# dioph/periodicity

Hardware: AMD Instinct MI355X
Metric: Lomb-Scargle Gpair/s (sample x freq), fp64, N=1e5 x 1e6 per GPU (higher is better)
Workload: dtype f64

## Files before the change

periodicity_amd/csrc/gls.hip:

```cpp
#include "pdc_internal.h"
#include "gls_epilogue.h"
#include "gls_sums.h"

#include <cstdlib>

using namespace pdc;

namespace {

constexpr int kBlock = 256;
constexpr int kPrepBlock = 1024;

enum Mode { MODE_FIT_MEAN = 0, MODE_NO_MEAN = 1, MODE_RAW = 2, MODE_TREND = 3 };
constexpr bool mode_fits_mean(int m) { return m == MODE_FIT_MEAN; }
constexpr bool mode_sums_w(int m) { return m == MODE_FIT_MEAN || m == MODE_TREND; }

struct TrendScalars {
    double W;
    double yy, y1, ty, tt, t1;
    double shift;
    double inv_span;
    double prec_a, prec_alpha, prec_beta;
    double log_const;
};
// ... 45 lines not shown
    const int64_t off = a.offsets ? a.offsets[blockIdx.x] : 0;
    const int64_t n = a.offsets ? a.offsets[blockIdx.x + 1] - off : a.n_total;
    const double *t = a.shared_t ? a.t : a.t + off;
    const int32_t *pk = a.picks ? a.picks + off : nullptr;
    const double *y = pk ? a.y : a.y + off;
    const double *dy = a.dy ? (pk ? a.dy : a.dy + off) : nullptr;
    auto at = [pk](int64_t i) -> int64_t { return pk ? (int64_t)pk[i] : i; };
    double *rec = a.rec + off * 6;
    const double t0 = n > 0 ? t[0] : 0.0;

    double W = 1.0, ybar = 0.0;
    if (!a.raw) {
        double acc = 0.0;
        for (int64_t i = tid; i < n; i += kPrepBlock) {
            const double e = dy ? dy[at(i)] : 1.0;
            acc += 1.0 / (e * e);
        }
        W = block_sum<kPrepBlock>(acc, red);
        if (a.fit_mean) {
            acc = 0.0;
            for (int64_t i = tid; i < n; i += kPrepBlock) {
                const double e = dy ? dy[at(i)] : 1.0;
                acc += (1.0 / (e * e)) / W * y[at(i)];
            }
            ybar = block_sum<kPrepBlock>(acc, red);
        }
    }
    double yy = 0.0, wsum = 0.0;
    if (a.rw) {
        for (int64_t i = tid; i < n; i += kPrepBlock) {
            const double e = dy ? dy[at(i)] : 1.0;
            const double w = (1.0 / (e * e)) / W;
            const double yc = y[at(i)] - ybar;
            const double wy = w * yc;
            yy += wy * yc;
            wsum += w;
            if (dy) reinterpret_cast<double2 *>(a.rw)[i * a.bpad + blockIdx.x] = make_double2(wy, w);
            else a.rw[i * a.bpad + blockIdx.x] = wy;
            if (blockIdx.x == 0) a.tp[i] = t[i] - t0;
        }
    } else
    for (int64_t i = tid; i < n; i += kPrepBlock) {
        const double tp = t[i] - t0;
        double w, wy;
        if (a.raw) {
            w = y[at(i)];
            wy = w;
        } else {
            const double e = dy ? dy[at(i)] : 1.0;
            w = (1.0 / (e * e)) / W;
            const double yc = y[at(i)] - ybar;
            wy = w * yc;
            yy += wy * yc;
            wsum += w;
        }
        double sd, cd;
        sincos_cycles(frac_product(a.delta, tp), sd, cd);
        if (!a.raw) {
            w = sqrt(w);
            wy = w * (y[at(i)] - ybar);
        }
        double2 *r = reinterpret_cast<double2 *>(rec + i * 6);
        r[0] = make_double2(wy, w);
        r[1] = make_double2(cd, sd);
        r[2] = make_double2(cd + cd, tp);
    }
    yy = block_sum<kPrepBlock>(yy, red);
    wsum = block_sum<kPrepBlock>(wsum, red);
    if (tid == 0) {
        double *s = a.scal + (int64_t)blockIdx.x * 4;
        s[0] = yy;
        s[1] = wsum;
        s[2] = W;
        s[3] = t0;
    }
}

constexpr int kPrepParts = 512;

struct WidePrepArgs {
    PrepArgs p;
    int nparts;
    double *part;
};

__global__ __launch_bounds__(kBlock) void gls_prep_wide_a(WidePrepArgs a) {
    __shared__ double red[kBlock / 64];
    double sw = 0.0, swy = 0.0;
    for (int64_t i = (int64_t)blockIdx.x * kBlock + threadIdx.x; i < a.p.n_total;
         i += (int64_t)gridDim.x * kBlock) {
        const double wr = inv_var(a.p.dy, i);
        sw += wr;
        swy += wr * a.p.y[i];
    }
    sw = block_sum<kBlock>(sw, red);
    swy = block_sum<kBlock>(swy, red);
    if (threadIdx.x == 0) {
        a.part[blockIdx.x] = sw;
        a.part[kPrepParts + blockIdx.x] = swy;
    }
}

__device__ __forceinline__ double fold_partials(const double *p, int count, double *red) {
    double v = 0.0;
    for (int i = threadIdx.x; i < count; i += kBlock) v += p[i];
    return block_sum<kBlock>(v, red);
}

__global__ __launch_bounds__(kBlock) void gls_prep_wide_b(WidePrepArgs a) {
    __shared__ double red[kBlock / 64];
    const double W = fold_partials(a.part, a.nparts, red);
    const double ybar = a.p.fit_mean ? fold_partials(a.part + kPrepParts, a.nparts, red) / W : 0.0;
    const double t0 = a.p.t[0];
    double yy = 0.0, wsum = 0.0;
    for (int64_t i = (int64_t)blockIdx.x * kBlock + threadIdx.x; i < a.p.n_total;
         i += (int64_t)gridDim.x * kBlock) {
        const double tp = a.p.t[i] - t0;
        const double w = inv_var(a.p.dy, i) / W;
        const double yc = a.p.y[i] - ybar;
        const double wy = w * yc;
        yy += wy * yc;
        wsum += w;
        double sd, cd;
        sincos_cycles(frac_product(a.p.delta, tp), sd, cd);
        const double rw = sqrt(w);
        double2 *r = reinterpret_cast<double2 *>(a.p.rec + i * 6);
        r[0] = make_double2(rw * yc, rw);
        r[1] = make_double2(cd, sd);
        r[2] = make_double2(cd + cd, tp);
    }
    yy = block_sum<kBlock>(yy, red);
    wsum = block_sum<kBlock>(wsum, red);
    if (threadIdx.x == 0) {
        a.part[2 * kPrepParts + blockIdx.x] = yy;
        a.part[3 * kPrepParts + blockIdx.x] = wsum;
    }
}

__global__ __launch_bounds__(kBlock) void gls_prep_wide_c(WidePrepArgs a) {
    __shared__ double red[kBlock / 64];
    const double W = fold_partials(a.part, a.nparts, red);
    const double yy = fold_partials(a.part + 2 * kPrepParts, a.nparts, red);
    const double wsum = fold_partials(a.part + 3 * kPrepParts, a.nparts, red);
    if (threadIdx.x == 0) {
        a.p.scal[0] = yy;
        a.p.scal[1] = wsum;
        a.p.scal[2] = W;
        a.p.scal[3] = a.p.t[0];
    }
}

constexpr int kPairM = 8;
constexpr int kPairRow = kPairM * 4;

__global__ __launch_bounds__(kBlock) void gls_pair_table_kernel(const double *rec, double *tab, int64_t n_total, double delta) {
    const int64_t g = (int64_t)blockIdx.x * kBlock + threadIdx.x;
    const int64_t i = g / kPairM;
    if (i >= n_total + 2) return;
    double c = 0.0, s = 0.0, c2 = 0.0, s2 = 0.0;
    if (i < n_total) {
        const double tp = rec[i * 6 + 5];
        const double k = (double)(2 * (int)(g % kPairM) + 1), h = 0.5 * delta;
        const double hi = h * tp, lo = __builtin_fma(h, tp, -hi);
        const double p = k * hi, pe = __builtin_fma(k, hi, -p);
        const double r = (p - __builtin_rint(p)) + __builtin_fma(k, lo, pe);
        sincos_cycles(r, s, c);
        sincos_cycles(r + r, s2, c2);
    }
    double2 *o = reinterpret_cast<double2 *>(tab + g * 4);
    o[0] = make_double2(c, s);
    o[1] = make_double2(c2, s2);
}

template <int MODE>
__device__ __forceinline__ double gls_power(double Sh, double Ch, double S, double C, double SS,
                                            double SC, double YY, double Wsum, double Werr,
                                            int psd) {
    const double S2 = 2.0 * SC;
    const double C2 = Wsum - 2.0 * SS;
    return gls_power_from_sums<mode_fits_mean(MODE)>(Sh, Ch, S, C, S2, C2, YY, Werr, psd);
}

__device__ __forceinline__ double bglst_loglik(double Sh, double Ch, double S, double C, double SS, double SC,
                                               double TS, double TC, double Wsum, const TrendScalars &q) {
    const double tc = TC * q.inv_span + q.shift * C, ts = TS * q.inv_span + q.shift * S;
    const double W = q.W;
    const double m00 = W * (Wsum - SS) + q.prec_a;
    const double m10 = W * SC, m11 = W * SS + q.prec_a;
    const double m20 = W * tc, m21 = W * ts, m22 = W * q.tt + q.prec_alpha;
    const double m30 = W * C, m31 = W * S, m32 = W * q.t1, m33 = W * Wsum + q.prec_beta;
    const double b0 = W * Ch, b1 = W * Sh, b2 = W * q.ty, b3 = W * q.y1;
    const double l00 = __builtin_sqrt(m00);
    const double l10 = m10 / l00, l20 = m20 / l00, l30 = m30 / l00;
    const double l11 = __builtin_sqrt(m11 - l10 * l10);
    const double l21 = (m21 - l20 * l10) / l11, l31 = (m31 - l30 * l10) / l11;
    const double l22 = __builtin_sqrt(m22 - l20 * l20 - l21 * l21);
    const double l32 = (m32 - l30 * l20 - l31 * l21) / l22;
    const double l33 = __builtin_sqrt(m33 - l30 * l30 - l31 * l31 - l32 * l32);
    const double z0 = b0 / l00;
    const double z1 = (b1 - l10 * z0) / l11;
    const double z2 = (b2 - l20 * z0 - l21 * z1) / l22;
    const double z3 = (b3 - l30 * z0 - l31 * z1 - l32 * z2) / l33;
    const double quad = W * q.yy - (z0 * z0 + z1 * z1 + z2 * z2 + z3 * z3);
    const double logdet = 2.0 * (log(l00) + log(l11) + log(l22) + log(l33));
    return -0.5 * (quad + logdet + q.log_const);
}

template <int K, int MODE, int SPLIT, bool BAL = false, bool PAIR = false>
__global__ __launch_bounds__(kBlock, (K >= 16 ? 2 : 1)) void gls_scan_kernel(GlsArgs a) {
    static_assert(!PAIR || (K == 2 * kPairM && (MODE == MODE_FIT_MEAN || MODE == MODE_NO_MEAN)), "mirrored pairs: K = 16, the two GLS modes");
    constexpr int FT = kBlock / SPLIT;
    constexpr bool TIGHT = BAL || K >= 16;
    constexpr int COLS = FT / 64;
    constexpr int kChunk = SPLIT == 1 ? 64 : 128;
    __shared__ double2 tab[kChunk + 1][COLS * 8 + 8 + 1];
    __shared__ double red_v[4];
    __shared__ long long red_i[4];
    __shared__ double2 sc_k[6];
    __shared__ double gf_red[PAIR ? 16 : 1][16];
    __shared__ double gf_acc[16];
    const int tid_ = threadIdx.x;
    if (TIGHT && tid_ < 6) sc_k[tid_] = sincos_coefficient(tid_);

    const int64_t G = BAL ? a.bal_slots : a.n_curves * a.tiles;
    const int64_t per_xcd = (G + 7) / 8;
    int64_t L = (int64_t)(blockIdx.x % 8) * per_xcd + blockIdx.x / 8;
    int zpart = blockIdx.y;
    if (a.parts_by_xcd) {
        const int64_t q = blockIdx.x / 8, zi = q / G;
        L = q - zi * G;
        zpart = (int)(blockIdx.x % 8) + 8 * (int)zi;
        if (zpart >= a.parts) return;
    }
    if (L >= G) return;
    int64_t bal_u = 0, bal_hi = 0;
    if (BAL) {
        bal_u = L * a.bal_units / a.bal_slots;
        bal_hi = (L + 1) * a.bal_units / a.bal_slots;
        if (bal_u >= bal_hi) return;
    }
    do {
    int64_t curve = L / a.tiles;
    int64_t tile = L - curve * a.tiles;
    int64_t bal_take = 0;
    int bal_piece = 0;
    int64_t bal_c0 = 0;
    if (BAL) {
        curve = 0;
        int64_t b_chunks = a.bal_chunks, b_slots = a.bal_slots, b_units = a.bal_units;
        asm volatile("" : "+s"(b_chunks), "+s"(b_slots), "+s"(b_units));
        tile = (bal_hi - 1) / b_chunks;
        const int64_t t0 = tile * b_chunks;
        bal_c0 = (bal_u > t0 ? bal_u : t0) - t0;
        bal_take = bal_hi - t0 - bal_c0;
        int64_t s_of = t0 * b_slots / b_units;
        while ((s_of + 1) * b_units / b_slots <= t0) ++s_of;
        while (s_of * b_units / b_slots > t0) --s_of;
        bal_piece = (int)(L - s_of);
    }

    const int64_t off = a.offsets ? a.offsets[curve] : 0;
    const int64_t n = a.offsets ? a.offsets[curve + 1] - off : a.n_total;
    const int wave = __builtin_amdgcn_readfirstlane(tid_ >> 6), part = wave % SPLIT;
    const int col = wave / SPLIT;
    const int64_t jt = tile * FT * (int64_t)K;
    const int64_t jl = jt + (col * 64 + (tid_ & 63)) * (int64_t)K;
    const double f_tile = __dadd_rn(a.f0, __dmul_rn((double)(a.j_begin + jt), a.delta));
    const double kdelta = (double)K * a.delta;

    static_assert(MODE != MODE_TREND || (SPLIT == 1 && !BAL && K <= 8), "BGLST: eight sums per frequency, whole curves per tile");
    double Sh[K], Ch[K], S[K], C[K], SS[K], SC[K];
    double TS[K], TC[K];
#pragma unroll
    for (int k = 0; k < K; ++k) Sh[k] = Ch[k] = S[k] = C[k] = SS[k] = SC[k] = TS[k] = TC[k] = 0.0;
    if (PAIR) {
        int t16 = tid_;
        asm volatile("" : "+v"(t16));
        if (t16 < 16) gf_acc[t16] = 0.0;
    }

    const int64_t s_begin = BAL ? bal_c0 * kChunk : (a.partial ? (int64_t)zpart * a.z_len : 0);
    const int64_t s_stop = BAL ? s_begin + bal_take * kChunk : s_begin + a.z_len;
    const int64_t s_end = (BAL || a.partial) ? (s_stop < n ? s_stop : n) : n;
    for (int64_t base = s_begin; base < s_end; base += kChunk) {
        __syncthreads();
        int tid = tid_;
        if (TIGHT) asm volatile("" : "+v"(tid));
        const int lane = tid & 63;
        const int slot_a = col * 8 + (lane >> 3), slot_b = COLS * 8 + (lane & 7);
        if (PAIR) {
            constexpr int SPP = kChunk / 16;
            const int m16 = tid & 15, seg = tid >> 4;
            const int64_t i0 = base + seg * SPP;
            const double *tp_ = a.pair_tab + (off + i0) * kPairRow + (m16 & 7) * 4 + (m16 < 8 ? 1 : 3);
            const double *rp_ = a.rec + (off + i0) * 6 + 1;
            double acc = 0.0;
#pragma unroll
            for (int q = 0; q < SPP; ++q) {
                const bool live = i0 + q < s_end;
                const double sq = live ? rp_[q * 6] : 0.0;
                const double v = live ? tp_[q * kPairRow] : 0.0;
                acc = __builtin_fma(sq * sq, m16 < 8 ? v * v : v, acc);
            }
            gf_red[seg][m16] = acc;
            __builtin_amdgcn_sched_barrier(0);
        }
        if (tid < 2 * kChunk) {
            const int il = tid >> 1;
            const bool live = base + il < s_end;
            const double tp = live ? a.rec[(off + base + il) * 6 + 5] : 0.0;
            const double sqw = live ? a.rec[(off + base + il) * 6 + 1] : 0.0;
            double2 step1, cur;
            double2 kk[6];
            if (TIGHT) {
#pragma unroll
                for (int q = 0; q < 6; ++q) kk[q] = sc_k[q];
            }
            auto sincos_fill = [&](const double r, double &s_, double &c_) {
                if (TIGHT) sincos_cycles_k(r, kk, s_, c_);
                else sincos_cycles(r, s_, c_);
            };
            if ((tid & 1) == 0) {
                sincos_fill(frac_product(kdelta, tp), step1.x, step1.y);
                double one = 1.0, zero = 0.0;
                if (TIGHT) asm volatile("" : "+v"(one), "+v"(zero));
                tab[il][COLS * 8] = make_double2(zero, one);
                tab[il][COLS * 8 + 1] = step1;
                cur = step1;
#pragma unroll
                for (int q = 2; q < 8; ++q) {
                    cur = rot2(cur, step1);
                    tab[il][COLS * 8 + q] = cur;
                }
                double r_base = frac_product(f_tile, tp);
                if (PAIR) {
                    double dl = a.delta;
                    asm volatile("" : "+v"(dl));
                    r_base += frac_product(8.0 * dl, tp) - frac_product(0.5 * dl, tp);
                }
                sincos_fill(r_base, cur.x, cur.y);
                if (MODE == MODE_FIT_MEAN || MODE == MODE_NO_MEAN || MODE == MODE_TREND) {
                    cur.x *= sqw;
                    cur.y *= sqw;
                }
            } else {
                sincos_fill(frac_product(8.0 * kdelta, tp), step1.x, step1.y);
            }
            double2 b0;
            b0.x = __shfl_xor(cur.x, 1, 64);
            b0.y = __shfl_xor(cur.y, 1, 64);
            if (tid & 1) {
                tab[il][0] = b0;
#pragma unroll
                for (int q = 1; q < COLS * 8; ++q) {
                    b0 = rot2(b0, step1);
                    tab[il][q] = b0;
                }
            }
        }
        __syncthreads();
        const int cnt = (int)((s_end - base) < kChunk ? (s_end - base) : kChunk);
        const int i_end = cnt < (part + 1) * (kChunk / SPLIT) ? cnt : (part + 1) * (kChunk / SPLIT);
        const int i_beg = part * (kChunk / SPLIT);
        if constexpr (PAIR) {
            if (tid < 16) {
                double g = gf_red[0][tid];
#pragma unroll
                for (int q = 1; q < 16; ++q) g += gf_red[q][tid];
                gf_acc[tid] += g;
            }
            using d8 = double __attribute__((ext_vector_type(8)));
            using cd8 = __attribute__((address_space(4))) const d8;
            using d2 = double __attribute__((ext_vector_type(2)));
            using cd2 = __attribute__((address_space(4))) const d2;
            auto uniform = [](const double *p) {
                const uintptr_t u = reinterpret_cast<uintptr_t>(p);
                const uint32_t lo_ = __builtin_amdgcn_readfirstlane((uint32_t)u), hi_ = __builtin_amdgcn_readfirstlane((uint32_t)(u >> 32));
                return ((uintptr_t)hi_ << 32) | lo_;
            };
            const cd8 *stab = reinterpret_cast<const cd8 *>(uniform(a.pair_tab + (off + base) * kPairRow));
            const cd2 *srec = reinterpret_cast<const cd2 *>(uniform(a.rec + (off + base) * 6));
            const int i_last = __builtin_amdgcn_readfirstlane(i_end);
            d8 h0a, h0b, h1a, h1b;
            d2 r;
            double2 qa, qt;
            auto request_first = [&](const int i) {
                h0a = stab[i * 4];
                h0b = stab[i * 4 + 1];
                r = srec[i * 3];
                qa = tab[i][slot_a];
                qt = tab[i][slot_b];
            };
            double A1, B1, A2, B2, a2, ab;
            auto pair_fmas = [&](const d8 &h, const int m0) {
#pragma unroll
                for (int q = 0; q < 2; ++q) {
                    const int hi = K / 2 + m0 + q, lo = K / 2 - 1 - m0 - q;
                    const double c = h[4 * q], s = h[4 * q + 1], c2 = h[4 * q + 2], s2 = h[4 * q + 3];
                    Sh[hi] = __builtin_fma(c, A1, Sh[hi]);
                    Sh[lo] = __builtin_fma(s, B1, Sh[lo]);
                    Ch[hi] = __builtin_fma(c, B1, Ch[hi]);
                    Ch[lo] = __builtin_fma(s, A1, Ch[lo]);
                    if (mode_sums_w(MODE)) {
                        S[hi] = __builtin_fma(c, A2, S[hi]);
                        S[lo] = __builtin_fma(s, B2, S[lo]);
                        C[hi] = __builtin_fma(c, B2, C[hi]);
                        C[lo] = __builtin_fma(s, A2, C[lo]);
                    }
                    SS[hi] = __builtin_fma(c2, a2, SS[hi]);
                    SS[lo] = __builtin_fma(s2, ab, SS[lo]);
                    SC[hi] = __builtin_fma(c2, ab, SC[hi]);
                    SC[lo] = __builtin_fma(s2, a2, SC[lo]);
                }
            };
            if (i_beg < i_last) {
                request_first(i_beg);
                for (int i = i_beg; i < i_last; ++i) {
                    __builtin_amdgcn_s_waitcnt(0xc07f);
                    h1a = stab[i * 4 + 2];
                    h1b = stab[i * 4 + 3];
                    __builtin_amdgcn_sched_barrier(0);
                    const double2 seed = rot2(qa, qt);
                    A1 = r[0] * seed.x;
                    B1 = r[0] * seed.y;
                    A2 = r[1] * seed.x;
                    B2 = r[1] * seed.y;
                    a2 = seed.x * seed.x;
                    ab = seed.x * seed.y;
                    pair_fmas(h0a, 0);
                    pair_fmas(h0b, 2);
                    __builtin_amdgcn_sched_barrier(0);
                    __builtin_amdgcn_s_waitcnt(0xc07f);
                    request_first(i + 1);
                    __builtin_amdgcn_sched_barrier(0);
                    pair_fmas(h1a, 4);
                    pair_fmas(h1b, 6);
                    __builtin_amdgcn_sched_barrier(0);
                }
            }
        } else {
        using d4 = double __attribute__((ext_vector_type(4)));
        using cd4 = __attribute__((address_space(4))) const d4;
        using cdbl = __attribute__((address_space(4))) const double;
        const cd4 *srec = reinterpret_cast<const cd4 *>(reinterpret_cast<uintptr_t>(a.rec + (off + base) * 6));
        struct Ahead {
            d4 r;
            double cd2;
            double tp;
            double2 qa, qt;
        };
        auto fetch = [&](const int i) {
            Ahead h;
            h.qa = tab[i][slot_a];
            h.qt = tab[i][slot_b];
            const cd4 *rp = reinterpret_cast<const cd4 *>(reinterpret_cast<const cdbl *>(srec) + i * 6);
            h.r = rp[0];
            h.cd2 = reinterpret_cast<const cdbl *>(rp)[4];
            h.tp = MODE == MODE_TREND ? reinterpret_cast<const cdbl *>(rp)[5] : 0.0;
            return h;
        };
        auto accumulate = [&](const Ahead &h) {
            const double2 seed = rot2(h.qa, h.qt);
            const double wy = h.r[0], w = h.r[1], cd = h.r[2], sd = h.r[3], cd2 = h.cd2;
            const double wt = MODE == MODE_TREND ? w * h.tp : 0.0;
            walk_grid<K>(seed, cd, sd, cd2, [&](const int k, const double s, const double c) {
                Sh[k] = __builtin_fma(wy, s, Sh[k]);
                Ch[k] = __builtin_fma(wy, c, Ch[k]);
                if (MODE != MODE_RAW) {
                    if (mode_sums_w(MODE)) {
                        S[k] = __builtin_fma(w, s, S[k]);
                        C[k] = __builtin_fma(w, c, C[k]);
                    }
                    if (MODE == MODE_TREND) {
                        TS[k] = __builtin_fma(wt, s, TS[k]);
                        TC[k] = __builtin_fma(wt, c, TC[k]);
                    }
                    SS[k] = __builtin_fma(s, s, SS[k]);
                    SC[k] = __builtin_fma(s, c, SC[k]);
                }
            });
        };
        Ahead A = fetch(i_beg);
        int i = i_beg;
        for (; i + 1 < i_end; i += 2) {
            __builtin_amdgcn_s_waitcnt(0xc07f);
            Ahead B = fetch(i + 1);
            __builtin_amdgcn_sched_barrier(0);
            accumulate(A);
            __builtin_amdgcn_sched_barrier(0);
            __builtin_amdgcn_s_waitcnt(0xc07f);
            A = fetch(i + 2);
            __builtin_amdgcn_sched_barrier(0);
            accumulate(B);
            __builtin_amdgcn_sched_barrier(0);
        }
        if (i < i_end) accumulate(A);
        }
    }

    if constexpr (PAIR) {
        __syncthreads();
        const bool keeps = part == 0;
#pragma unroll
        for (int m = 0; m < K / 2; ++m) {
            const int hi = K / 2 + m, lo = K / 2 - 1 - m;
            const double G = keeps ? gf_acc[m] : 0.0, Fh = keeps ? 0.5 * gf_acc[8 + m] : 0.0;
            double p = Sh[hi], q = Sh[lo];
            Sh[hi] = p + q;
            Sh[lo] = p - q;
            p = Ch[hi], q = Ch[lo];
            Ch[hi] = p - q;
            Ch[lo] = p + q;
            if (mode_sums_w(MODE)) {
                p = S[hi], q = S[lo];
                S[hi] = p + q;
                S[lo] = p - q;
                p = C[hi], q = C[lo];
                C[hi] = p - q;
                C[lo] = p + q;
            }
            p = SS[hi] + G, q = SS[lo];
            SS[hi] = p + q;
            SS[lo] = p - q;
            p = SC[hi], q = Fh - SC[lo];
            SC[hi] = p + q;
            SC[lo] = p - q;
            asm volatile("" : "+v"(Sh[hi]), "+v"(Sh[lo]), "+v"(Ch[hi]), "+v"(Ch[lo]), "+v"(SS[hi]), "+v"(SS[lo]), "+v"(SC[hi]), "+v"(SC[lo]));
            if (mode_sums_w(MODE)) asm volatile("" : "+v"(S[hi]), "+v"(S[lo]), "+v"(C[hi]), "+v"(C[lo]));
            __builtin_amdgcn_sched_barrier(0);
        }
        __syncthreads();
    }

    const int tid = tid_;
    if (SPLIT > 1) {
        double *xch = reinterpret_cast<double *>(tab);
        const int slot = ((wave / SPLIT) * (SPLIT - 1) + (part - 1)) * 64 + (tid & 63);
#pragma unroll
        for (int k = 0; k < K; ++k) {
            __syncthreads();
            if (part > 0) {
                double *d = xch + slot * 6;
                d[0] = Sh[k]; d[1] = Ch[k]; d[2] = S[k]; d[3] = C[k]; d[4] = SS[k]; d[5] = SC[k];
            }
            __syncthreads();
            if (part == 0) {
#pragma unroll
                for (int q = 0; q < SPLIT - 1; ++q) {
                    const double *d = xch + (((wave / SPLIT) * (SPLIT - 1) + q) * 64 + (tid & 63)) * 6;
                    Sh[k] += d[0]; Ch[k] += d[1]; S[k] += d[2]; C[k] += d[3]; SS[k] += d[4]; SC[k] += d[5];
                }
            }
        }
    }
    const bool owner = part == 0;

    if (MODE != MODE_RAW && (BAL || a.partial)) {
        double *out = a.partial + (int64_t)(BAL ? bal_piece : zpart) * 6 * a.nf;
        auto put = [&](const double (&v)[K], const int q) {
#pragma unroll
            for (int k = 0; k < K; ++k)
                if (owner && jl + k < a.nf) out[(int64_t)q * a.nf + jl + k] = v[k];
        };
        put(Sh, 0);
        put(Ch, 1);
        put(S, 2);
        put(C, 3);
        put(SS, 4);
        put(SC, 5);
        if (BAL) {
            bal_hi -= bal_take;
            continue;
        }
// ... 369 lines not shown
            }
        };
        w8 a0 = wrow[0], a1 = wrow[1];
        double2 ta[4], tb[4];
#pragma unroll
        for (int k = 0; k < 4; ++k) ta[k] = trig[0][k][lane];
        for (int il = 0; il < cnt; il += 2) {
            __builtin_amdgcn_s_waitcnt(0xc07f);
            const w8 b0 = wrow[wstride], b1 = wrow[wstride + 1];
#pragma unroll
            for (int k = 0; k < 4; ++k) tb[k] = trig[il + 1][k][lane];
            __builtin_amdgcn_sched_barrier(0);
            accumulate(a0, a1, ta);
            __builtin_amdgcn_sched_barrier(0);
            __builtin_amdgcn_s_waitcnt(0xc07f);
            a0 = wrow[2 * wstride];
            a1 = wrow[2 * wstride + 1];
#pragma unroll
            for (int k = 0; k < 4; ++k) ta[k] = trig[il + 2][k][lane];
            __builtin_amdgcn_sched_barrier(0);
            accumulate(b0, b1, tb);
            __builtin_amdgcn_sched_barrier(0);
            wrow += 2 * wstride;
        }
    }

    const int64_t tiles64 = (a.nf + 63) / 64;
#pragma unroll
    for (int r = 0; r < RT; ++r) {
        const int64_t b = r0 + r;
        if (b >= a.n_curves) break;
        const double *sc = a.scal + b * 4;
        const double YY = sc[0], Wsum = sc[1], Werr = sc[2];
#pragma unroll
        for (int h = 0; h < 2; ++h) {
            const int64_t j = h ? jb : ja;
            const bool valid = j < a.nf;
            const double p = gls_power<MODE>(Sh[h][r], Ch[h][r], S[h][r], C[h][r], SS[h][r], SC[h][r], YY, Wsum, Werr, a.psd);
            if (valid && a.power) a.power[b * a.nf + j] = p;
            if (a.blk_max && 2 * tile + h < tiles64) {
                double best = 0.0;
                long long best_j = -1;
                if (valid && p == p) {
                    best = p;
                    best_j = j;
                }
#pragma unroll
                for (int o = 32; o > 0; o >>= 1) {
                    const double ov = __shfl_down(best, o, 64);
                    const long long oj = __shfl_down(best_j, o, 64);
                    if (oj >= 0 && (best_j < 0 || ov > best || (ov == best && oj < best_j))) {
                        best = ov;
                        best_j = oj;
                    }
                }
                if (lane == 0) {
                    a.blk_max[b * tiles64 + 2 * tile + h] = best;
                    a.blk_arg[b * tiles64 + 2 * tile + h] = best_j;
                }
            }
        }
    }
}

__global__ __launch_bounds__(64) void gls_peak_kernel(const double *blk_max, const int64_t *blk_arg,
                                                      int64_t tiles, double *amax, int64_t *argmax) {
    const int64_t curve = blockIdx.x;
    double best = 0.0;
    long long best_j = -1;
    for (int64_t i = threadIdx.x; i < tiles; i += 64) {
        const double v = blk_max[curve * tiles + i];
        const long long j = blk_arg[curve * tiles + i];
        if (j >= 0 && (best_j < 0 || v > best)) {
            best = v;
            best_j = j;
        }
    }
#pragma unroll
    for (int o = 32; o > 0; o >>= 1) {
        const double ov = __shfl_down(best, o, 64);
        const long long oj = __shfl_down(best_j, o, 64);
        if (oj >= 0 && (best_j < 0 || ov > best || (ov == best && oj < best_j))) {
            best = ov;
            best_j = oj;
        }
    }
    if (threadIdx.x == 0) {
        if (amax) amax[curve] = best_j >= 0 ? best : __builtin_nan("");
        if (argmax) argmax[curve] = best_j;
    }
}

constexpr int64_t kPartialCells = (int64_t)1 << 20;
constexpr int kPartsMax = 512;

void tile_shape(int64_t n_curves, int64_t nf, int64_t n_total, bool may_split, int *K_out, int *S_out, int *Z_out) {
    static const int envK = [] { const char *e = getenv("PDC_GLS_K"); return e ? atoi(e) : 0; }();
    static const int envS = [] { const char *e = getenv("PDC_GLS_S"); return e ? atoi(e) : 0; }();
    static const int envZ = [] { const char *e = getenv("PDC_GLS_Z"); return e ? atoi(e) : 0; }();
    int64_t z_max = 1;
    if (may_split && n_curves == 1 && n_total >= 16384) {
        z_max = n_total / 2048;
        const int64_t room = kPartialCells / (nf > 0 ? nf : 1);
        z_max = z_max < room ? z_max : room;
        z_max = z_max > kPartsMax ? kPartsMax : (z_max < 1 ? 1 : z_max);
    }
    double best = 1e300;
    int bk = 8, bs = 1, bz = 1;
    for (int K : {16, 8, 4}) {
        if (envK && K != envK) continue;
        for (int S : {1, 2, 4}) {
            if (envS && S != envS) continue;
            const double tile_waves = (double)n_curves * (double)((nf + 64 * K - 1) / (64 * K)) * S;
            int64_t Z = (int64_t)__builtin_ceil(2048.0 / tile_waves);
            Z = Z > z_max ? z_max : (Z < 1 ? 1 : Z);
            if (Z >= 8) Z -= Z % 8;
            if (envZ) Z = envZ > z_max ? z_max : envZ;
            const double waves = tile_waves * (double)Z;
            const double rounds = __builtin_ceil(waves / 1024.0);
            double cost = rounds * (12.0 + 8.0 * K) / ((double)S * (double)Z);
            if (waves / 1024.0 <= 1.0) cost *= 1.10;
            cost *= 1.0 + 0.02 * (S > 2 ? S - 2 : 2 - S);
            if (Z > 1) cost *= 1.02;
            if (cost < best) {
                best = cost;
                bk = K;
                bs = S;
                bz = (int)Z;
            }
        }
    }
    *K_out = bk;
    *S_out = bs;
    *Z_out = bz;
}

template <int MODE, int S>
void launch_scan_ks(int K, dim3 grid, hipStream_t st, const GlsArgs &a) {
    if constexpr (MODE == MODE_FIT_MEAN || MODE == MODE_NO_MEAN) {
        if (K == 16 && a.pair_tab) {
            hipLaunchKernelGGL((gls_scan_kernel<16, MODE, S, false, true>), grid, dim3(kBlock), 0, st, a);
            return;
        }
    }
    switch (K) {
        case 4: hipLaunchKernelGGL((gls_scan_kernel<4, MODE, S>), grid, dim3(kBlock), 0, st, a); break;
        case 16: hipLaunchKernelGGL((gls_scan_kernel<16, MODE, S>), grid, dim3(kBlock), 0, st, a); break;
        default: hipLaunchKernelGGL((gls_scan_kernel<8, MODE, S>), grid, dim3(kBlock), 0, st, a); break;
    }
}

template <int MODE>
void launch_scan_balanced(int S, dim3 grid, hipStream_t st, const GlsArgs &a) {
    if (a.pair_tab) {
        if (S == 2) hipLaunchKernelGGL((gls_scan_kernel<16, MODE, 2, true, true>), grid, dim3(kBlock), 0, st, a);
        else hipLaunchKernelGGL((gls_scan_kernel<16, MODE, 4, true, true>), grid, dim3(kBlock), 0, st, a);
    } else {
        if (S == 2) hipLaunchKernelGGL((gls_scan_kernel<16, MODE, 2, true>), grid, dim3(kBlock), 0, st, a);
        else hipLaunchKernelGGL((gls_scan_kernel<16, MODE, 4, true>), grid, dim3(kBlock), 0, st, a);
    }
}

template <int MODE>
void launch_scan(int K, int S, dim3 grid, hipStream_t st, const GlsArgs &a) {
    switch (S) {
        case 4: launch_scan_ks<MODE, 4>(K, grid, st, a); break;
        case 2: launch_scan_ks<MODE, 2>(K, grid, st, a); break;
        default: launch_scan_ks<MODE, 1>(K, grid, st, a); break;
    }
}

struct WorkLayout {
    int64_t rec, scal, parts, blk_max, blk_arg, partial, pair, total;
};

enum Route { ROUTE_NONE = 0, ROUTE_GENERAL = 1, ROUTE_PARTS = 2, ROUTE_BALANCED = 3, ROUTE_SHARED = 4, ROUTE_SHARED2 = 5 };
struct Dispatch {
    int64_t route, K, S, tiles, parts, parts_by_xcd, bal_slots, wide_prep, bpad, groups, z_len, bal_chunks;
};
thread_local Dispatch g_last_dispatch = {};
struct PairUse {
    int64_t ran, table_bytes;
};
thread_local PairUse g_last_pair = {};

WorkLayout layout(int64_t n_total, int64_t n_curves, int64_t nf) {
    auto up = [](int64_t x) { return (x + 255) & ~(int64_t)255; };
    const int64_t tiles_max = (nf + 63) / 64;
    WorkLayout w;
    w.rec = 0;
    w.scal = up(n_total * 48);
    w.parts = w.scal + up(n_curves * 32);
    w.blk_max = w.parts + up(4 * kPrepParts * 8);
    w.blk_arg = w.blk_max + up(n_curves * tiles_max * 8);
    w.partial = w.blk_arg + up(n_curves * tiles_max * 8);
    int64_t cells = kPartsMax * nf < kPartialCells ? kPartsMax * nf : kPartialCells;
    cells = cells > 3 * nf ? cells : 3 * nf;
    w.pair = w.partial + (n_curves == 1 ? up(cells * 6 * 8) : 0);
    w.total = w.pair + up((n_total + 2) * kPairRow * 8);
    return w;
}

int scan_dev(int device, hipStream_t st, const double *d_t, const double *d_y, const double *d_dy,
             const int64_t *d_offsets, int64_t n_total, int64_t n_curves, int shared_t, double f0,
             double delta, int64_t j_begin, int64_t nf, int mode, int psd, double *d_power,
             double *d_raw_s, double *d_raw_c, double *d_amax, int64_t *d_argmax, void *work,
             int64_t work_bytes, const int32_t *d_picks = nullptr, const TrendScalars *trend = nullptr) {
    PDC_REQUIRE(d_t && d_y, "gls: t and y must not be NULL");
    PDC_REQUIRE((mode == MODE_TREND) == (trend != nullptr) && (mode != MODE_TREND || (n_curves == 1 && !d_picks && !shared_t)),
                "gls: the trend mode takes one curve and its scalars");
    PDC_REQUIRE(!d_picks || (shared_t && d_offsets && mode != MODE_RAW), "gls: picks need a shared time axis");
    PDC_REQUIRE(n_total >= 0 && n_curves >= 1 && nf >= 0 && j_begin >= 0, "gls: negative size");
    PDC_REQUIRE(n_curves == 1 || d_offsets, "gls: a batch needs offsets");
    PDC_REQUIRE(n_curves * ((nf + 255) / 256 + 1) < (int64_t)1 << 31, "gls: grid too large");
    const WorkLayout w = layout(n_total, n_curves, nf);
    PDC_REQUIRE(work && work_bytes >= w.total, "gls: workspace too small (%lld < %lld bytes)",
                (long long)work_bytes, (long long)w.total);
    if (nf == 0) return PDC_OK;
    PDC_TRY(use_device(device));
    char *base = static_cast<char *>(work);
    Dispatch &rec = g_last_dispatch;
    rec = Dispatch{};
    rec.parts = 1;
    g_last_pair = PairUse{};

    PrepArgs p;
    p.t = d_t;
    p.y = d_y;
    p.dy = d_dy;
    p.offsets = d_offsets;
    p.n_total = n_total;
    p.shared_t = shared_t;
    p.fit_mean = mode == MODE_FIT_MEAN;
    p.raw = mode == MODE_RAW;
    p.delta = delta;
    p.rec = reinterpret_cast<double *>(base + w.rec);
    p.scal = reinterpret_cast<double *>(base + w.scal);
    p.picks = d_picks;
    const bool peaks = d_amax || d_argmax;

    static const int env_shared = [] { const char *e = getenv("PDC_GLS_SHARED"); return e ? atoi(e) : -1; }();
    if (shared_t && mode != MODE_RAW && n_curves >= 2 && env_shared != 0) {
        const bool uni = d_dy == nullptr;
        const int64_t n = n_total / n_curves;
        const int64_t group = (int64_t)kShWaves * (uni ? kShCurvesU : kShCurvesW);
        const int64_t bpad = (n_curves + group - 1) / group * group;
        const int64_t table = (n + 2) * bpad * (uni ? 8 : 16);
        if ((n_curves >= 96 || env_shared == 1) && table + n * 8 <= w.scal && n * n_curves == n_total) {
            p.rw = p.rec;
            p.tp = reinterpret_cast<double *>(base + table);
            p.bpad = bpad;
            PDC_HIP(hipMemsetAsync(base + table / (n + 2) * n, 0, table / (n + 2) * 2, st));
            hipLaunchKernelGGL(gls_prep_kernel, dim3((unsigned)n_curves), dim3(kPrepBlock), 0, st, p);
            PDC_HIP(hipGetLastError());
            SharedArgs sa;
            sa.tp = p.tp;
            sa.rw = p.rw;
            sa.scal = p.scal;
            sa.n = n;
            sa.n_curves = n_curves;
            sa.bpad = bpad;
            sa.tiles = (nf + 63) / 64;
            sa.groups = bpad / group;
            sa.f0 = f0;
            sa.delta = delta;
            sa.j_begin = j_begin;
            sa.nf = nf;
            sa.psd = psd;
            sa.power = d_power;
            sa.blk_max = peaks ? reinterpret_cast<double *>(base + w.blk_max) : nullptr;
            sa.blk_arg = peaks ? reinterpret_cast<int64_t *>(base + w.blk_arg) : nullptr;
            static const bool sh2 = [] { const char *e = getenv("PDC_GLS_SH2"); return !(e && e[0] == '0'); }();
            if (!uni && sh2) {
                sa.groups = bpad / (kSh2Waves * kSh2Curves);
                const int64_t G2 = sa.groups * ((nf + 127) / 128);
                PDC_REQUIRE(G2 < (int64_t)1 << 31, "gls: grid too large");
                const dim3 grid2((unsigned)(((G2 + 7) / 8) * 8));
                rec.route = ROUTE_SHARED2;
                rec.K = 2;
                rec.tiles = (nf + 127) / 128;
                rec.bpad = bpad;
                rec.groups = sa.groups;
                if (mode == MODE_FIT_MEAN) {
                    PDC_TRY(allow_dynamic_lds((const void *)gls_shared2_kernel<true>, (int)kSh2Lds));
                    hipLaunchKernelGGL((gls_shared2_kernel<true>), grid2, dim3(kSh2Block), kSh2Lds, st, sa);
                } else {
                    PDC_TRY(allow_dynamic_lds((const void *)gls_shared2_kernel<false>, (int)kSh2Lds));
                    hipLaunchKernelGGL((gls_shared2_kernel<false>), grid2, dim3(kSh2Block), kSh2Lds, st, sa);
                }
                PDC_HIP(hipGetLastError());
                if (peaks) {
                    hipLaunchKernelGGL(gls_peak_kernel, dim3((unsigned)n_curves), dim3(64), 0, st, sa.blk_max,
                                       sa.blk_arg, sa.tiles, d_amax, d_argmax);
                    PDC_HIP(hipGetLastError());
                }
                return PDC_OK;
            }
            const int64_t G = sa.groups * sa.tiles;
            PDC_REQUIRE(G < (int64_t)1 << 31, "gls: grid too large");
            const dim3 grid((unsigned)(((G + 7) / 8) * 8));
            rec.route = ROUTE_SHARED;
            rec.K = 1;
            rec.tiles = sa.tiles;
            rec.bpad = bpad;
            rec.groups = sa.groups;
            if (mode == MODE_FIT_MEAN) {
                if (uni) hipLaunchKernelGGL((gls_shared_kernel<true, true>), grid, dim3(kShBlock), 0, st, sa);
// ... 295 lines not shown
```

Measured before the change: 4189.

## Prefetch next pair-table chunk and restructure pair-mode sincos table fill

Adds a read-ahead in the mirrored-pair scan kernel that touches the next chunk's pair table and sample records while the current chunk is processed, warming the cache ahead of the scalar loads. It also rewrites the pair-mode twiddle-table fill so odd and even lanes split the work: one lane builds the base-phase rotations and the other builds the step rotations. The sample loads for that fill are moved earlier. For large balanced grids (more than 512 slots) it instead dispatches a variant with the read-ahead disabled, and it adds compile-time knockout switches for experiments. The cost is extra load instructions and more template instances, and the new phase computation may change rounding.

```diff
diff --git a/periodicity_amd/csrc/gls.hip b/periodicity_amd/csrc/gls.hip
--- a/periodicity_amd/csrc/gls.hip
+++ b/periodicity_amd/csrc/gls.hip
@@ -221,6 +221,10 @@
 
 constexpr int kPairM = 8;
 constexpr int kPairRow = kPairM * 4;
+#ifndef PDC_GLS_PAIR_KNOCKOUT
+#define PDC_GLS_PAIR_KNOCKOUT 0
+#endif
+constexpr int kPairKnockout = PDC_GLS_PAIR_KNOCKOUT;
 
 __global__ __launch_bounds__(kBlock) void gls_pair_table_kernel(const double *rec, double *tab, int64_t n_total, double delta) {
     const int64_t g = (int64_t)blockIdx.x * kBlock + threadIdx.x;
@@ -275,8 +279,12 @@
     return -0.5 * (quad + logdet + q.log_const);
 }
 
-template <int K, int MODE, int SPLIT, bool BAL = false, bool PAIR = false>
+constexpr int kNoAhead = 8;
+template <int K, int MODE, int SPLIT_, bool BAL = false, bool PAIR = false>
 __global__ __launch_bounds__(kBlock, (K >= 16 ? 2 : 1)) void gls_scan_kernel(GlsArgs a) {
+    constexpr int SPLIT = SPLIT_ & (kNoAhead - 1);
+    constexpr bool AHEAD = PAIR && !(SPLIT_ & kNoAhead);
+    static_assert(SPLIT_ == SPLIT || (SPLIT_ == SPLIT + kNoAhead && BAL && PAIR), "no read-ahead: a variant of the balanced pair instances");
     static_assert(!PAIR || (K == 2 * kPairM && (MODE == MODE_FIT_MEAN || MODE == MODE_NO_MEAN)), "mirrored pairs: K = 16, the two GLS modes");
     constexpr int FT = kBlock / SPLIT;
     constexpr bool TIGHT = BAL || K >= 16;
@@ -344,20 +352,32 @@
     for (int k = 0; k < K; ++k) Sh[k] = Ch[k] = S[k] = C[k] = SS[k] = SC[k] = TS[k] = TC[k] = 0.0;
     if (PAIR) {
         int t16 = tid_;
-        asm volatile("" : "+v"(t16));
-        if (t16 < 16) gf_acc[t16] = 0.0;
+        double zero = 0.0;
+        asm volatile("" : "+v"(t16), "+v"(zero));
+        if (t16 < 16) gf_acc[t16] = zero;
     }
 
     const int64_t s_begin = BAL ? bal_c0 * kChunk : (a.partial ? (int64_t)zpart * a.z_len : 0);
     const int64_t s_stop = BAL ? s_begin + bal_take * kChunk : s_begin + a.z_len;
     const int64_t s_end = (BAL || a.partial) ? (s_stop < n ? s_stop : n) : n;
+    unsigned ahead_tab = 0, ahead_rec = 0;
     for (int64_t base = s_begin; base < s_end; base += kChunk) {
-        __syncthreads();
+        if (AHEAD) asm volatile("" : : "v"(ahead_tab), "v"(ahead_rec));
+        const bool seam = !(PAIR && kPairKnockout >= 2) || base == s_begin;
+        const bool sync = !(PAIR && kPairKnockout >= 3) || base == s_begin;
+        if (sync) __syncthreads();
         int tid = tid_;
         if (TIGHT) asm volatile("" : "+v"(tid));
         const int lane = tid & 63;
         const int slot_a = col * 8 + (lane >> 3), slot_b = COLS * 8 + (lane & 7);
-        if (PAIR) {
+        double fill_tp = 0.0, fill_sqw = 0.0;
+        if (PAIR && seam && tid < 2 * kChunk) {
+            const int il = tid >> 1;
+            const bool live = base + il < s_end;
+            fill_tp = live ? a.rec[(off + base + il) * 6 + 5] : 0.0;
+            fill_sqw = live ? a.rec[(off + base + il) * 6 + 1] : 0.0;
+        }
+        if (PAIR && seam) {
             constexpr int SPP = kChunk / 16;
             const int m16 = tid & 15, seg = tid >> 4;
             const int64_t i0 = base + seg * SPP;
@@ -374,11 +394,11 @@
             gf_red[seg][m16] = acc;
             __builtin_amdgcn_sched_barrier(0);
         }
-        if (tid < 2 * kChunk) {
+        if (seam && tid < 2 * kChunk) {
             const int il = tid >> 1;
             const bool live = base + il < s_end;
-            const double tp = live ? a.rec[(off + base + il) * 6 + 5] : 0.0;
-            const double sqw = live ? a.rec[(off + base + il) * 6 + 1] : 0.0;
+            const double tp = PAIR ? fill_tp : (live ? a.rec[(off + base + il) * 6 + 5] : 0.0);
+            const double sqw = PAIR ? fill_sqw : (live ? a.rec[(off + base + il) * 6 + 1] : 0.0);
             double2 step1, cur;
             double2 kk[6];
             if (TIGHT) {
@@ -389,6 +409,31 @@
                 if (TIGHT) sincos_cycles_k(r, kk, s_, c_);
                 else sincos_cycles(r, s_, c_);
             };
+            if constexpr (PAIR) {
+                const bool odd = tid & 1;
+                sincos_fill(frac_product(odd ? 8.0 * kdelta : kdelta, tp), step1.x, step1.y);
+                double dl = a.delta;
+                asm volatile("" : "+v"(dl));
+                const double r_base = frac_product(f_tile, tp) + (frac_product(8.0 * dl, tp) - frac_product(0.5 * dl, tp));
+                sincos_fill(r_base, cur.x, cur.y);
+                cur.x *= sqw;
+                cur.y *= sqw;
+                if (odd) {
+                    tab[il][0] = cur;
+                } else {
+                    double one = 1.0, zero = 0.0;
+                    asm volatile("" : "+v"(one), "+v"(zero));
+                    tab[il][COLS * 8] = make_double2(zero, one);
+                    tab[il][COLS * 8 + 1] = step1;
+                    cur = step1;
+                }
+#pragma unroll
+                for (int q = 1; q < COLS * 8; ++q) {
+                    cur = rot2(cur, step1);
+                    if (odd) tab[il][q] = cur;
+                    else if (q + 1 < 8) tab[il][COLS * 8 + q + 1] = cur;
+                }
+            } else {
             if ((tid & 1) == 0) {
                 sincos_fill(frac_product(kdelta, tp), step1.x, step1.y);
                 double one = 1.0, zero = 0.0;
@@ -426,27 +471,38 @@
                     tab[il][q] = b0;
                 }
             }
-        }
-        __syncthreads();
+            }
+        }
+        if (sync) __syncthreads();
         const int cnt = (int)((s_end - base) < kChunk ? (s_end - base) : kChunk);
         const int i_end = cnt < (part + 1) * (kChunk / SPLIT) ? cnt : (part + 1) * (kChunk / SPLIT);
         const int i_beg = part * (kChunk / SPLIT);
         if constexpr (PAIR) {
-            if (tid < 16) {
+            if (seam && tid < 16) {
                 double g = gf_red[0][tid];
 #pragma unroll
                 for (int q = 1; q < 16; ++q) g += gf_red[q][tid];
                 gf_acc[tid] += g;
             }
-            using d8 = double __attribute__((ext_vector_type(8)));
-            using cd8 = __attribute__((address_space(4))) const d8;
-            using d2 = double __attribute__((ext_vector_type(2)));
-            using cd2 = __attribute__((address_space(4))) const d2;
             auto uniform = [](const double *p) {
                 const uintptr_t u = reinterpret_cast<uintptr_t>(p);
                 const uint32_t lo_ = __builtin_amdgcn_readfirstlane((uint32_t)u), hi_ = __builtin_amdgcn_readfirstlane((uint32_t)(u >> 32));
                 return ((uintptr_t)hi_ << 32) | lo_;
             };
+            if (AHEAD && base + kChunk < s_end) {
+                const int64_t nb = base + kChunk;
+                const unsigned left = __builtin_amdgcn_readfirstlane((unsigned)(s_end - nb < kChunk ? s_end - nb : kChunk));
+                const unsigned t_bytes = (left + 2 < kChunk ? left + 2 : kChunk) * (kPairRow * 8), r_bytes = left * 48;
+                const unsigned o = (unsigned)tid * 128;
+                const char *tb = reinterpret_cast<const char *>(uniform(a.pair_tab + (off + nb) * kPairRow));
+                const char *rb = reinterpret_cast<const char *>(uniform(a.rec + (off + nb) * 6));
+                if (o < t_bytes) ahead_tab = *reinterpret_cast<const unsigned *>(tb + o);
+                if (o < r_bytes + 128) ahead_rec = *reinterpret_cast<const unsigned *>(rb + (o < r_bytes - 8 ? o : r_bytes - 8));
+            }
+            using d8 = double __attribute__((ext_vector_type(8)));
+            using cd8 = __attribute__((address_space(4))) const d8;
+            using d2 = double __attribute__((ext_vector_type(2)));
+            using cd2 = __attribute__((address_space(4))) const d2;
             const cd8 *stab = reinterpret_cast<const cd8 *>(uniform(a.pair_tab + (off + base) * kPairRow));
             const cd2 *srec = reinterpret_cast<const cd2 *>(uniform(a.rec + (off + base) * 6));
             const int i_last = __builtin_amdgcn_readfirstlane(i_end);
@@ -454,9 +510,10 @@
             d2 r;
             double2 qa, qt;
             auto request_first = [&](const int i) {
-                h0a = stab[i * 4];
-                h0b = stab[i * 4 + 1];
-                r = srec[i * 3];
+                const int ir = kPairKnockout == 1 ? 0 : i;
+                h0a = stab[ir * 4];
+                h0b = stab[ir * 4 + 1];
+                r = srec[ir * 3];
                 qa = tab[i][slot_a];
                 qt = tab[i][slot_b];
             };
@@ -486,8 +543,8 @@
                 request_first(i_beg);
                 for (int i = i_beg; i < i_last; ++i) {
                     __builtin_amdgcn_s_waitcnt(0xc07f);
-                    h1a = stab[i * 4 + 2];
-                    h1b = stab[i * 4 + 3];
+                    h1a = stab[(kPairKnockout == 1 ? 0 : i) * 4 + 2];
+                    h1b = stab[(kPairKnockout == 1 ? 0 : i) * 4 + 3];
                     __builtin_amdgcn_sched_barrier(0);
                     const double2 seed = rot2(qa, qt);
                     A1 = r[0] * seed.x;
@@ -1163,7 +1220,10 @@
 
 template <int MODE>
 void launch_scan_balanced(int S, dim3 grid, hipStream_t st, const GlsArgs &a) {
-    if (a.pair_tab) {
+    if (a.pair_tab && a.bal_slots > 512) {
+        if (S == 2) hipLaunchKernelGGL((gls_scan_kernel<16, MODE, 2 + kNoAhead, true, true>), grid, dim3(kBlock), 0, st, a);
+        else hipLaunchKernelGGL((gls_scan_kernel<16, MODE, 4 + kNoAhead, true, true>), grid, dim3(kBlock), 0, st, a);
+    } else if (a.pair_tab) {
         if (S == 2) hipLaunchKernelGGL((gls_scan_kernel<16, MODE, 2, true, true>), grid, dim3(kBlock), 0, st, a);
         else hipLaunchKernelGGL((gls_scan_kernel<16, MODE, 4, true, true>), grid, dim3(kBlock), 0, st, a);
     } else {
```

Result: no change. 4221 (median of 6 runs) (+0.8%).
